# yoraish/mmd

Hardware: AMD Instinct MI355X
Metric: guided trajectories/sec (H=64, 100 denoise steps), 32-robot Empty map (higher is better)
Workload: dtype f32 (f16x2 split on the fp16 MFMA pipe: every fp32 product as 3 fp16 MFMAs, fp32 accumulate)

## Files before the change

mmd_amd/csrc/guide.hip:

```cpp
#include <hip/hip_runtime.h>

#include <atomic>
#include <cmath>

#include "../../include/mmd_amd.h"
#include "../../include/mmd_amd_debug.h"
#include "bins_dev.h"
#include "common.h"
#include "guide_dev.h"

namespace mmd {

__device__ __forceinline__ float clip_scale(float gx, float gy, float gz, float gw, float max_norm) {
  const float ax = gx + 1e-6f, ay = gy + 1e-6f, az = gz + 1e-6f, aw = gw + 1e-6f;
  const float n2 = ax * ax + ay * ay + az * az + aw * aw;
  return fminf(max_norm * __builtin_amdgcn_rsqf(n2), 1.f);
}

__device__ __forceinline__ bool clip_grad(const GuideDev& g, float& gx, float& gy, float& gz, float& gw) {
  if (g.clip_rule == 0) {
    const float sc = clip_scale(gx, gy, gz, gw, g.max_norm);
    gx = sc * gx; gy = sc * gy; gz = sc * gz; gw = sc * gw;
    return sc < 1.f;
  } else if (g.clip_rule == 1) {
    const float m = g.max_value;
    const bool on = fabsf(gx) > m || fabsf(gy) > m || fabsf(gz) > m || fabsf(gw) > m;
    gx = fminf(fmaxf(gx, -m), m); gy = fminf(fmaxf(gy, -m), m); gz = fminf(fmaxf(gz, -m), m); gw = fminf(fmaxf(gw, -m), m);
    return on;
  }
  return false;
}
__device__ __forceinline__ bool clip_grad(const GuideDev& g, float& gx, float& gy) {
  float z = 0.f, w = 0.f;
  return clip_grad(g, gx, gy, z, w);
}

__device__ __forceinline__ float lane_prev(float v) {
  return __builtin_bit_cast(float, __builtin_amdgcn_update_dpp(0, __builtin_bit_cast(int, v), 0x138, 0xf, 0xf, true));
}
__device__ __forceinline__ float lane_next(float v) {
  return __builtin_bit_cast(float, __builtin_amdgcn_update_dpp(0, __builtin_bit_cast(int, v), 0x130, 0xf, 0xf, true));
}

constexpr int LDS_SLOTS_SMALL = 40;
constexpr int LDS_SLOTS_MAX = 144;

__device__ __forceinline__ float rsq_pos(float d2) { return __builtin_amdgcn_rsqf(fmaxf(d2, 1e-30f)); }

typedef float f32x2g __attribute__((ext_vector_type(2)));
struct Acc4 { f32x2g a0, a1, a2, a3; };
__device__ __forceinline__ Acc4 acc4_zero() {
  const f32x2g z = {0.f, 0.f};
  return Acc4{z, z, z, z};
}
__device__ __forceinline__ f32x2g acc4_total(const Acc4& r) {
  return f32x2g{(r.a0.x + r.a1.x) + (r.a2.x + r.a3.x), (r.a0.y + r.a1.y) + (r.a2.y + r.a3.y)};
}
__device__ __forceinline__ f32x2g cons_term(f32x2g a, f32x2g p, f32x2g q, float r2) {
  const float dx = p.x - q.x, dy = p.y - q.y;
  const float d2 = __builtin_fmaf(dx, dx, dy * dy);
  const float m = (d2 > r2) ? 0.f : rsq_pos(d2);
  return f32x2g{__builtin_fmaf(-dx, m, a.x), __builtin_fmaf(-dy, m, a.y)};
}
template <bool COMPACT> struct ConsTab;
template <> struct ConsTab<false> {
  const float4* tab;
  float r2;
  __device__ __forceinline__ f32x2g add(f32x2g a, f32x2g p, int slot, int t) const {
    const float4 c = tab[slot * H + t];
    return cons_term(a, p, f32x2g{c.x, c.y}, c.w);
  }
};
template <> struct ConsTab<true> {
  const float2* tab;
  float r2;
  __device__ __forceinline__ f32x2g add(f32x2g a, f32x2g p, int slot, int t) const {
    const float2 c = tab[slot * H + t];
    return cons_term(a, p, f32x2g{c.x, c.y}, r2);
  }
};
template <class TAB>
__device__ __forceinline__ void cons_accumulate4(Acc4& acc, const TAB& tab, int first, int n, int rel, int t, f32x2g p) {
  auto one = [&](int k, int slot) {
    if (k == 0) acc.a0 = tab.add(acc.a0, p, slot, t);
    else if (k == 1) acc.a1 = tab.add(acc.a1, p, slot, t);
    else if (k == 2) acc.a2 = tab.add(acc.a2, p, slot, t);
    else acc.a3 = tab.add(acc.a3, p, slot, t);
  };
  int i = 0;
  for (; i < n && ((rel + i) & 3); ++i) one((rel + i) & 3, first + i);
#pragma unroll 2
  for (; i + 3 < n; i += 4) {
    acc.a0 = tab.add(acc.a0, p, first + i, t);
    acc.a1 = tab.add(acc.a1, p, first + i + 1, t);
    acc.a2 = tab.add(acc.a2, p, first + i + 2, t);
    acc.a3 = tab.add(acc.a3, p, first + i + 3, t);
  }
  for (int k = 0; i < n; ++i, ++k) one(k, first + i);
}
template <class TAB>
__device__ __forceinline__ f32x2g cons_accumulate1(f32x2g a, const TAB& tab, int first, int n, int rel, int k, int t, f32x2g p) {
#pragma unroll 4
  for (int j = (k - rel) & 3; j < n; j += 4) a = tab.add(a, p, first + j, t);
  return a;
}

struct GroupMeta {
  static constexpr bool kOneGroup = false;
  int s0[2], s1[2];
  float w[2];
  int grp0, n;
  __device__ __forceinline__ void load(const GuideDev& g, int g0, int g1) {
    grp0 = g0;
    n = min(g1 - g0, 2);
#pragma unroll
    for (int k = 0; k < 2; ++k) {
      s0[k] = s1[k] = 0;
      w[k] = 0.f;
      if (k < n) {
        s0[k] = __builtin_amdgcn_readfirstlane(g.grp_slot_off[g0 + k]);
        s1[k] = __builtin_amdgcn_readfirstlane(g.grp_slot_off[g0 + k + 1]);
        w[k] = __builtin_bit_cast(float, __builtin_amdgcn_readfirstlane(__builtin_bit_cast(int, g.grp_weight[g0 + k])));
      }
    }
  }
  __device__ __forceinline__ void bounds(const GuideDev& g, int grp, int& a, int& b) const {
    const int k = grp - grp0;
    if (k == 0 && n > 0) { a = s0[0]; b = s1[0]; }
    else if (k == 1 && n > 1) { a = s0[1]; b = s1[1]; }
    else { a = __builtin_amdgcn_readfirstlane(g.grp_slot_off[grp]); b = __builtin_amdgcn_readfirstlane(g.grp_slot_off[grp + 1]); }
  }
  __device__ __forceinline__ float weight(const GuideDev& g, int grp) const {
    const int k = grp - grp0;
    return (k == 0 && n > 0) ? w[0] : (k == 1 && n > 1) ? w[1] : g.grp_weight[grp];
  }
};

template <bool DUMP = false, class GROUPSUM, class GROUPW>
__device__ __forceinline__ float4 guide_grad(const GuideDev& g, float4 xn, int t, const float4* __restrict__ grid,
                                             int grp0, int grp1, GROUPSUM group_sum, GROUPW group_weight, unsigned int* tr = nullptr) {
  unsigned int flags = 0;
  float xu[4];
  const float xv[4] = {xn.x, xn.y, xn.z, xn.w};
#pragma unroll
  for (int d = 0; d < 4; ++d) {
    float v = fminf(fmaxf(xv[d], -1.f), 1.f);
    if constexpr (DUMP) flags |= (fabsf(xv[d]) > 1.f ? 1u : 0u) << (16 + d);
    v = (v + 1.f) / 2.f;
    xu[d] = v * g.nscale[d] + g.nmin[d];
  }
  const float px = xu[0], py = xu[1], vx = xu[2], vy = xu[3];
  const bool interior = t > 0 && t < H - 1;

  int ix = (int)floorf((px - g.lo[0]) / g.dim[0] * (float)g.nx);
  int iy = (int)floorf((py - g.lo[1]) / g.dim[1] * (float)g.ny);
  ix = min(max(ix, 0), g.nx - 1);
  iy = min(max(iy, 0), g.ny - 1);
  const float4 cell0 = g.n_grids > 0 ? grid[(size_t)ix * g.ny + iy] : make_float4(1e30f, 0.f, 0.f, 0.f);

  float wsx, wsy;
  {
    const float d0 = px - g.ws_min[0], d1 = py - g.ws_min[1], d2 = g.ws_max[0] - px, d3 = g.ws_max[1] - py;
    float best = fmaxf(g.margin - d0, 0.f), gx = -1.f, gy = 0.f;
    float v = fmaxf(g.margin - d1, 0.f);
    if (v > best) { best = v; gx = 0.f; gy = -1.f; }
    v = fmaxf(g.margin - d2, 0.f);
    if (v > best) { best = v; gx = 1.f; gy = 0.f; }
    v = fmaxf(g.margin - d3, 0.f);
    if (v > best) { best = v; gx = 0.f; gy = 1.f; }
    if (!(best > 0.f)) { gx = 0.f; gy = 0.f; }
    if constexpr (DUMP) {
      const unsigned arg = gx < 0.f ? 0u : gy < 0.f ? 1u : gx > 0.f ? 2u : 3u;
      if (best > 0.f) flags |= 1u << 4 | arg << 5;
    }
    const bool clipped = clip_grad(g, gx, gy);
    if constexpr (DUMP) flags |= (clipped ? 1u : 0u) << 9;
    wsx = g.w_coll * gx; wsy = g.w_coll * gy;
  }
  float gpx, gpy, gpz, gpw;
  {
    const float npx = lane_next(px), npy = lane_next(py), nvx = lane_next(vx), nvy = lane_next(vy);
    float wpx = 0.f, wpy = 0.f, wvx = 0.f, wvy = 0.f;
    if (t < H - 1) {
      const float epx = npx - (px + g.dt * vx), epy = npy - (py + g.dt * vy);
      const float evx = nvx - vx, evy = nvy - vy;
      wpx = 2.f * (g.m1 * epx + g.m2 * evx);
      wpy = 2.f * (g.m1 * epy + g.m2 * evy);
      wvx = 2.f * (g.m2 * epx + g.m3 * evx);
      wvy = 2.f * (g.m2 * epy + g.m3 * evy);
    }
    const float lpx = lane_prev(wpx), lpy = lane_prev(wpy), lvx = lane_prev(wvx), lvy = lane_prev(wvy);
    float gx = lpx - wpx, gy = lpy - wpy;
    float gz = lvx - (g.dt * wpx + wvx), gw = lvy - (g.dt * wpy + wvy);
    const bool clipped = clip_grad(g, gx, gy, gz, gw);
    if constexpr (DUMP) flags |= (clipped ? 1u : 0u) << 10;
    gpx = g.w_smooth * gx; gpy = g.w_smooth * gy;
    gpz = g.w_smooth * gz; gpw = g.w_smooth * gw;
  }
  float cx = 0.f, cy = 0.f;
  for (int grp = grp0; grp < grp1; ++grp) {
    const f32x2g gs = group_sum(grp, f32x2g{px, py});
    float gx = gs.x, gy = gs.y;
    const bool clipped = clip_grad(g, gx, gy);
    if constexpr (DUMP) {
      const int k = grp - grp0, s0 = g.grp_slot_off[grp], s1 = g.grp_slot_off[grp + 1];
      unsigned long long mask = 0;
      unsigned int n_act = 0;
      for (int sl = s0; sl < s1; ++sl) {
        const float4 c = g.cons[(size_t)sl * H + t];
        const float dx = px - c.x, dy = py - c.y;
        const float d2 = __builtin_fmaf(dx, dx, dy * dy);
        if (!(d2 > c.w)) {
          ++n_act;
          if (sl - s0 < 64) mask |= 1ull << (sl - s0);
        }
      }
      if (k < 4) {
        tr[2 + 2 * k] = (unsigned int)mask;
        tr[3 + 2 * k] = (unsigned int)(mask >> 32);
        flags |= (clipped ? 1u : 0u) << (11 + k);
      }
      tr[10] += n_act;
    }
    const float w = group_weight(grp);
    cx += w * gx; cy += w * gy;
  }
  float ox, oy;
  {
    float best = fmaxf(g.margin - cell0.x, 0.f), gx = 0.f, gy = 0.f;
    unsigned win = 0;
    if (best > 0.f) { gx = -cell0.y; gy = -cell0.z; }
    for (int k = 1; k < g.n_grids; ++k) {
      const float4 c = grid[((size_t)k * g.nx + ix) * g.ny + iy];
      const float v = fmaxf(g.margin - c.x, 0.f);
      if (v > best) { best = v; gx = -c.y; gy = -c.z; win = (unsigned)k; }
    }
    if (g.n_xs + g.n_xb > 0) {
      float ex, ey;
      const float v = fmaxf(g.margin - extra_sdf(g.xs, g.n_xs, g.xb, g.n_xb, px, py, ex, ey), 0.f);
      if (v > best) { best = v; gx = -ex; gy = -ey; win = 7u; }
    }
    const bool clipped = clip_grad(g, gx, gy);
    if constexpr (DUMP) {
      if (best > 0.f) flags |= 1u | (win & 7u) << 1;
      flags |= (clipped ? 1u : 0u) << 8;
    }
    ox = g.w_coll * gx; oy = g.w_coll * gy;
  }
  if constexpr (DUMP) {
    tr[0] = (unsigned int)(ix * g.ny + iy);
    tr[1] = flags | (unsigned int)min(grp1 - grp0, 15) << 20;
  }
  float tx = ((ox + wsx) + gpx) + cx, ty = ((oy + wsy) + gpy) + cy;
  float tz = gpz, tw = gpw;
  if (!interior) { tx = ty = tz = tw = 0.f; }
  return make_float4(-tx, -ty, -tz, -tw);
}


template <bool COMPACT, int NT>
__device__ __forceinline__ void stage_cons(const GuideDev& g, int robot, int lds_slots, float4* lds_cons, int& lds_slot0, int& lds_n) {
  lds_slot0 = __builtin_amdgcn_readfirstlane(g.grp_slot_off[g.robot_grp_off[robot]]);
  lds_n = min(__builtin_amdgcn_readfirstlane(g.grp_slot_off[g.robot_grp_off[robot + 1]]) - lds_slot0, lds_slots);
  const float4* src = g.cons + (size_t)lds_slot0 * H;
  if constexpr (COMPACT) {
    float2* dst = reinterpret_cast<float2*>(lds_cons);
    for (int i = threadIdx.x; i < lds_n * H; i += NT) {
      const float4 c = src[i];
      dst[i] = c.z < 0.f ? make_float2(1e30f, 1e30f) : make_float2(c.x, c.y);
    }
  } else {
    for (int i = threadIdx.x; i < lds_n * H; i += NT) lds_cons[i] = src[i];
  }
}

template <bool COMPACT, class ACC>
__device__ __forceinline__ void group_slots(const GuideDev& g, const GroupMeta& gm, int grp, const float4* lds_cons, int lds_slot0, int lds_n,
                                            ACC acc) {
  int s0, s1;
  gm.bounds(g, grp, s0, s1);
  const int l0 = min(max(s0 - lds_slot0, 0), lds_n), l1 = min(max(s1 - lds_slot0, 0), lds_n);
  if (l1 > l0) {
    if constexpr (COMPACT) acc(ConsTab<true>{reinterpret_cast<const float2*>(lds_cons), g.uniform_r2}, l0, l1 - l0, lds_slot0 + l0 - s0);
    else acc(ConsTab<false>{lds_cons, 0.f}, l0, l1 - l0, lds_slot0 + l0 - s0);
  }
  const int g0 = lds_n > 0 ? max(s0, lds_slot0 + lds_n) : s0;
  if (s1 > g0) acc(ConsTab<false>{g.cons, 0.f}, g0, s1 - g0, g0 - s0);
}

__device__ __forceinline__ float4 model_update(StepDev s, float4 v, const float4* eps, size_t idx) {
  if (s.do_model)
    v = s.ddim == 2 ? ddim_update_x0(v, eps[idx], s.a_t, s.b_t, s.c1, s.c2)
        : s.ddim ? ddim_update(v, eps[idx], s.a_t, s.b_t, s.c1, s.c2) : ddpm_posterior_mean(v, eps[idx], s.a_t, s.b_t, s.c1, s.c2);
  return v;
}

template <bool DUMP, class META = GroupMeta, class GROUPSUM>
__device__ __forceinline__ void guide_iterations(const GuideDev& g, const StepDev& s, int robot, int t, size_t idx, float4& v, bool is_hard,
                                                 float4 hv, bool store, GROUPSUM group_sum) {
  const int map = g.robot_map ? g.robot_map[robot] : 0;
  const float4* grid = g.grids + (size_t)map * g.n_grids * g.nx * g.ny;
  int grp0 = 0, grp1 = 0;
  if constexpr (META::kOneGroup) {
    grp1 = 1;
  } else if (g.robot_grp_off) {
    grp0 = __builtin_amdgcn_readfirstlane(g.robot_grp_off[robot]);
    grp1 = __builtin_amdgcn_readfirstlane(g.robot_grp_off[robot + 1]);
  }
  META gm;
  if constexpr (META::kOneGroup) gm.w = group_sum.weight;
  gm.load(g, grp0, grp1);
  for (int it = 0; it < s.n_guide_steps; ++it) {
    unsigned int* tr = nullptr;
    if constexpr (DUMP) {
      tr = s.trace + ((size_t)it * s.guide_chain_stride + idx) * MMD_TRACE_WORDS;
      for (int w = 0; w < MMD_TRACE_WORDS; ++w) tr[w] = 0u;
    }
    const float4 gr = guide_grad<DUMP>(g, v, t, grid, grp0, grp1, [&](int grp, f32x2g p) { return group_sum(gm, grp, p); },
                                       [&](int grp) { return gm.weight(g, grp); }, tr);
    v.x = __builtin_fmaf(s.grad_scale, gr.x, v.x); v.y = __builtin_fmaf(s.grad_scale, gr.y, v.y);
    v.z = __builtin_fmaf(s.grad_scale, gr.z, v.z); v.w = __builtin_fmaf(s.grad_scale, gr.w, v.w);
    if (is_hard) v = hv;
    if (s.guide_chain && store) s.guide_chain[(size_t)it * s.guide_chain_stride + idx] = v;
  }
}

__device__ __forceinline__ void step_finish(const StepDev& s, float4* x, const float4* noise, float4* chain, size_t idx, int robot,
                                            int samples_per_robot, float4& v, bool is_hard, const float4& hv) {
  if (s.do_noise) v = add_step_noise(v, noise ? noise[idx] : traj_normal4(s.seed, s.robot_seeds, s.draw, s.traj_base, idx, robot, samples_per_robot), s.sigma, s.noise_std_extra);
  if (is_hard) v = hv;
  x[idx] = v;
  if (chain) chain[idx] = v;
}

template <int WPB, bool COMPACT, bool DUMP = false>
__global__ __launch_bounds__(WPB * 64) void ddpm_guide_kernel(GuideDev g, StepDev s, int lds_slots, float4* __restrict__ x,
                                                         const float4* __restrict__ eps,
                                                         const float4* __restrict__ noise, float4* __restrict__ chain,
                                                         const float4* __restrict__ hard,
                                                         int samples_per_robot) {
  extern __shared__ __attribute__((aligned(16))) float4 lds_cons[];
  const int t = threadIdx.x & 63;
  const int traj_b = s.traj0 + blockIdx.x * WPB;
  const int traj = traj_b + (threadIdx.x >> 6);
  const bool valid = traj < s.traj_end;

  int lds_slot0 = 0, lds_n = 0;
  if (s.do_guide && g.robot_grp_off) {
    const int rb0 = traj_b / samples_per_robot;
    const int rb1 = min(traj_b + WPB - 1, s.traj_end - 1) / samples_per_robot;
    if (rb0 == rb1) stage_cons<COMPACT, WPB * 64>(g, rb0, lds_slots, lds_cons, lds_slot0, lds_n);
  }
  __syncthreads();
  if (!valid) return;

  const int robot = traj / samples_per_robot;
  const size_t idx = (size_t)traj * H + t;
  float4 v = model_update(s, x[idx], eps, idx);
  float4 hv = v;
  const bool is_hard = hard_row(s.hard_rows, s.n_hard, hard, robot, t, hv);
  if constexpr (DUMP) {
    if (s.mu_out) s.mu_out[idx] = v;
  }
  if (s.do_guide)
    guide_iterations<DUMP>(g, s, robot, t, idx, v, is_hard, hv, true, [&](const GroupMeta& gm, int grp, f32x2g p) {
      Acc4 acc = acc4_zero();
      group_slots<COMPACT>(g, gm, grp, lds_cons, lds_slot0, lds_n,
                           [&](const auto& tab, int first, int n, int rel) { cons_accumulate4(acc, tab, first, n, rel, t, p); });
      return acc4_total(acc);
    });
  step_finish(s, x, noise, chain, idx, robot, samples_per_robot, v, is_hard, hv);
}

constexpr int COOP_XCH_BYTES = 2 * 4 * H * 8;
template <bool COMPACT>
__global__ __launch_bounds__(256) void ddpm_guide_coop_kernel(GuideDev g, StepDev s, int lds_slots, float4* __restrict__ x,
                                                              const float4* __restrict__ eps, const float4* __restrict__ noise,
                                                              float4* __restrict__ chain, const float4* __restrict__ hard,
                                                              int samples_per_robot) {
  extern __shared__ __attribute__((aligned(16))) float4 lds_cons[];
  const int t = threadIdx.x & 63, wave = __builtin_amdgcn_readfirstlane(threadIdx.x >> 6);
  const int traj = s.traj0 + blockIdx.x;
  const int robot = traj / samples_per_robot;
  float2* const xch = reinterpret_cast<float2*>(reinterpret_cast<char*>(lds_cons) + (size_t)lds_slots * H * (COMPACT ? 8 : 16));
  int lds_slot0 = 0, lds_n = 0;
  if (s.do_guide && g.robot_grp_off) stage_cons<COMPACT, 256>(g, robot, lds_slots, lds_cons, lds_slot0, lds_n);
  __syncthreads();
  const size_t idx = (size_t)traj * H + t;
  float4 v = model_update(s, x[idx], eps, idx);
  float4 hv = v;
  const bool is_hard = hard_row(s.hard_rows, s.n_hard, hard, robot, t, hv);
  if (s.do_guide) {
    int parity = 0;
    guide_iterations<false>(g, s, robot, t, idx, v, is_hard, hv, wave == 0, [&](const GroupMeta& gm, int grp, f32x2g p) {
      f32x2g a = {0.f, 0.f};
      group_slots<COMPACT>(g, gm, grp, lds_cons, lds_slot0, lds_n,
                           [&](const auto& tab, int first, int n, int rel) { a = cons_accumulate1(a, tab, first, n, rel, wave, t, p); });
      float2* const slot = xch + parity * 4 * H;
      slot[wave * H + t] = make_float2(a.x, a.y);
      __syncthreads();
      parity ^= 1;
      const float2 q0 = slot[t], q1 = slot[H + t], q2 = slot[2 * H + t], q3 = slot[3 * H + t];
      return acc4_total(Acc4{f32x2g{q0.x, q0.y}, f32x2g{q1.x, q1.y}, f32x2g{q2.x, q2.y}, f32x2g{q3.x, q3.y}});
    });
  }
  if (wave != 0) return;
  step_finish(s, x, noise, chain, idx, robot, samples_per_robot, v, is_hard, hv);
}


struct OneGroup {
  static constexpr bool kOneGroup = true;
  float w;
  __device__ __forceinline__ void load(const GuideDev&, int, int) {}
  __device__ __forceinline__ float weight(const GuideDev&, int) const { return w; }
};

struct BinnedSum {
  const mmd_cons_bins& b;
  int t, self;
  float r2, weight;
  __device__ __forceinline__ f32x2g operator()(const OneGroup&, int, f32x2g p) const {
    const CellList cl = own_cell_list(b, t, p.x, p.y);
    const float4 none = make_float4(0.f, 0.f, __builtin_bit_cast(float, self), 0.f);
    Acc4 acc = acc4_zero();
    const int last = max(cl.e1 - 1, 0);
    for (int e = cl.e0; __builtin_amdgcn_ballot_w64(e < cl.e1) != 0; e += 4) {
      float4 c[4];
#pragma unroll
      for (int j = 0; j < 4; ++j) {
        const float4 l = cl.ent[min(e + j, last)];
        c[j] = e + j < cl.e1 ? l : none;
      }
#pragma unroll
      for (int j = 0; j < 4; ++j) {
        const int id = __builtin_bit_cast(int, c[j].z);
        const int k = (id - (id > self ? 1 : 0)) & 3;
        f32x2g a = k == 0 ? acc.a0 : k == 1 ? acc.a1 : k == 2 ? acc.a2 : acc.a3;
        a = cons_term(a, p, f32x2g{c[j].x, c[j].y}, id != self ? r2 : -1.f);
        acc.a0 = k == 0 ? a : acc.a0;
        acc.a1 = k == 1 ? a : acc.a1;
        acc.a2 = k == 2 ? a : acc.a2;
        acc.a3 = k == 3 ? a : acc.a3;
      }
    }
    return acc4_total(acc);
  }
};

__global__ __launch_bounds__(256) void ddpm_guide_binned_kernel(GuideDev g, StepDev s, mmd_cons_bins b, float4* __restrict__ x,
                                                                const float4* __restrict__ eps, const float4* __restrict__ noise,
                                                                float4* __restrict__ chain, const float4* __restrict__ hard,
                                                                int samples_per_robot) {
  const int t = threadIdx.x & 63;
  const int traj = s.traj0 + blockIdx.x * 4 + (threadIdx.x >> 6);
  if (traj >= s.traj_end) return;
  const int robot = traj / samples_per_robot;
  const size_t idx = (size_t)traj * H + t;
  float4 v = model_update(s, x[idx], eps, idx);
  float4 hv = v;
  const bool is_hard = hard_row(s.hard_rows, s.n_hard, hard, robot, t, hv);
  if (s.do_guide)
    guide_iterations<false, OneGroup>(g, s, robot, t, idx, v, is_hard, hv, true,
                                      BinnedSum{b, t, b.robot0 + robot, b.radius * fabsf(b.radius), b.weight});
  step_finish(s, x, noise, chain, idx, robot, samples_per_robot, v, is_hard, hv);
}

__global__ void init_kernel(float4* __restrict__ x, float4* __restrict__ chain, const float4* __restrict__ hard,
                            unsigned long long hard_rows, int draw_noise, unsigned long long seed,
                            const unsigned long long* __restrict__ robot_seeds, long long traj_base, int n_traj, int samples_per_robot) {
  const size_t idx = (size_t)blockIdx.x * blockDim.x + threadIdx.x;
  if (idx >= (size_t)n_traj * H) return;
  const int t = idx % H;
  const int robot = (idx / H) / samples_per_robot;
  float4 v = draw_noise ? traj_normal4(seed, robot_seeds, 0xFFFFFFFFu, traj_base, idx, robot, samples_per_robot) : x[idx];
  float4 hv;
  if (hard_row(hard_rows, __popcll(hard_rows), hard, robot, t, hv)) v = hv;
  x[idx] = v;
  if (chain) chain[idx] = v;
}

__global__ void q_sample_kernel(float4* __restrict__ x, const float4* __restrict__ x0, const float4* __restrict__ noise,
                                float a, float b, unsigned long long seed, unsigned int draw, long long traj_base,
                                size_t n_pts) {
  const size_t idx = (size_t)blockIdx.x * blockDim.x + threadIdx.x;
  if (idx >= n_pts) return;
  const float4 z = noise ? noise[idx] : normal4(seed, draw, (unsigned long long)traj_base * H + idx);
  const float4 s = x0[idx];
  x[idx] = make_float4(a * s.x + b * z.x, a * s.y + b * z.y, a * s.z + b * z.z, a * s.w + b * z.w);
}

__global__ void cross_condition_kernel(float4* __restrict__ x1, float4* __restrict__ x2, float4* __restrict__ c1,
                                       float4* __restrict__ c2, int ind1, int ind2, float4 rel, float4 bnd,
                                       const float4* __restrict__ by_robot, int spr, int n_traj) {
  const int b = blockIdx.x * blockDim.x + threadIdx.x;
  if (b >= n_traj) return;
  if (by_robot) {
    rel = by_robot[(size_t)(b / spr) * 2];
    bnd = by_robot[(size_t)(b / spr) * 2 + 1];
  }
  const float4 v2 = x2[(size_t)b * H + ind2];
  float4 v1;
  v1.x = fminf(v2.x + rel.x, bnd.x); v1.y = fminf(v2.y + rel.y, bnd.y);
  v1.z = fminf(v2.z + rel.z, bnd.z); v1.w = fminf(v2.w + rel.w, bnd.w);
  x1[(size_t)b * H + ind1] = v1;
  float4 w;
  w.x = fmaxf(v1.x - rel.x, -bnd.x); w.y = fmaxf(v1.y - rel.y, -bnd.y);
  w.z = fmaxf(v1.z - rel.z, -bnd.z); w.w = fmaxf(v1.w - rel.w, -bnd.w);
  x2[(size_t)b * H + ind2] = w;
  if (c1) c1[(size_t)b * H + ind1] = v1;
  if (c2) c2[(size_t)b * H + ind2] = w;
}

int fill_guide(const mmd_guide_desc* d, GuideDev& g) {
  MMD_REQUIRE(d->n_grids == 0 || (d->sdf_grids_dev && d->grid_nx >= 1 && d->grid_ny >= 1), "guide: SDF grid missing");
  if (d->cons_bins) {
    MMD_REQUIRE(!d->cons_ell_dev, "guide: cons_bins together with an ELL table (cons_ell_dev) is not supported");
    if (int rc = check_cons_bins(d->cons_bins)) return rc;
  }
  for (int k = 0; k < 4; ++k) { g.nmin[k] = d->norm_min[k]; g.nscale[k] = d->norm_max[k] - d->norm_min[k]; }
  for (int k = 0; k < 2; ++k) {
    g.lo[k] = d->limits_lo[k];
    g.dim[k] = fabsf(d->limits_hi[k] - d->limits_lo[k]);
    g.ws_min[k] = d->ws_min[k]; g.ws_max[k] = d->ws_max[k];
  }
  g.nx = d->grid_nx; g.ny = d->grid_ny; g.n_grids = d->n_grids;
  g.grids = reinterpret_cast<const float4*>(d->sdf_grids_dev);
  g.robot_map = d->robot_map_dev;
  g.margin = d->margin; g.dt = d->dt; g.w_coll = d->weight_collision; g.w_smooth = d->weight_smoothness;
  g.max_norm = d->max_grad_norm;
  MMD_REQUIRE(d->clip_grad_rule >= 0 && d->clip_grad_rule <= 2, "guide: clip_grad_rule must be 0 (norm), 1 (value) or 2 (off)");
  g.clip_rule = d->clip_grad_rule;
  g.max_value = d->max_grad_value;
  const double dt = d->dt, qc = 1.0 / ((double)d->sigma_gp * d->sigma_gp);
  g.m1 = (float)(12.0 / (dt * dt * dt) * qc);
  g.m2 = (float)(-6.0 / (dt * dt) * qc);
  g.m3 = (float)(4.0 / dt * qc);
  g.max_slots = d->max_slots_per_robot > 0 ? d->max_slots_per_robot : LDS_SLOTS_SMALL;
  g.uniform_r2 = d->cons_uniform_radius > 0.f ? d->cons_uniform_radius * fabsf(d->cons_uniform_radius) : 0.f;
  g.xs = reinterpret_cast<const float4*>(d->extra_spheres_dev); g.n_xs = d->extra_spheres_dev ? d->n_extra_spheres : 0;
  g.xb = reinterpret_cast<const float4*>(d->extra_boxes_dev); g.n_xb = d->extra_boxes_dev ? d->n_extra_boxes : 0;
  g.cons = reinterpret_cast<const float4*>(d->cons_ell_dev);
  g.grp_slot_off = d->grp_slot_off_dev; g.grp_weight = d->grp_weight_dev; g.robot_grp_off = d->robot_grp_off_dev;
  if (!g.cons || !g.grp_slot_off || !g.grp_weight) g.robot_grp_off = nullptr;
  return 0;
}

constexpr int kCoopMaxTrajDefault = 512;

int launch_step(const GuideDev& g, StepDev s, float* x, const float* eps, const float* noise, float* chain,
                const float* hard, int traj0, int n_traj, int spr, hipStream_t st, const mmd_cons_bins* bins) {
  s.traj0 = traj0;
  s.traj_end = traj0 + n_traj;
  if (bins && s.do_guide) {
    hipLaunchKernelGGL(ddpm_guide_binned_kernel, dim3((n_traj + 3) / 4), dim3(256), 0, st, g, s, *bins, (float4*)x, (const float4*)eps,
                       (const float4*)noise, (float4*)chain, (const float4*)hard, spr);
    return 0;
  }
  const bool guided = s.do_guide && g.robot_grp_off;
  const bool compact = guided && g.uniform_r2 > 0.f;
  const int bytes_per_slot = H * (compact ? 8 : 16);
  const int small = LDS_SLOTS_SMALL * (compact ? 2 : 1), big = LDS_SLOTS_MAX * (compact ? 2 : 1);
  auto launch = [&](auto kern, int grid, int block, size_t lds_bytes, int slots) {
    hipLaunchKernelGGL(kern, dim3(grid), dim3(block), lds_bytes, st, g, s, slots, (float4*)x, (const float4*)eps, (const float4*)noise,
                       (float4*)chain, (const float4*)hard, spr);
  };
  if (s.trace) {
    launch(ddpm_guide_kernel<4, false, true>, (n_traj + 3) / 4, 256, 0, 0);
  } else if (guided && n_traj <= (s.coop_max > 0 ? s.coop_max : s.coop_max < 0 ? 0 : kCoopMaxTrajDefault)) {
    const int fit = 60 * 1024 / bytes_per_slot;
    const int slots = g.max_slots < fit ? g.max_slots : fit;
    launch(compact ? ddpm_guide_coop_kernel<true> : ddpm_guide_coop_kernel<false>, n_traj, 256,
           (size_t)slots * bytes_per_slot + COOP_XCH_BYTES, slots);
  } else if (guided && g.max_slots > small && spr % 8 == 0 && traj0 % 8 == 0) {
    const int slots = g.max_slots < big ? g.max_slots : big;
    static std::atomic<unsigned long long> attr_devices{0};
    int dev = 0;
    (void)hipGetDevice(&dev);
    const unsigned long long bit = 1ull << (dev & 63);
    if (!(attr_devices.load(std::memory_order_acquire) & bit)) {
      (void)hipFuncSetAttribute(reinterpret_cast<const void*>(&ddpm_guide_kernel<8, false>),
                                hipFuncAttributeMaxDynamicSharedMemorySize, LDS_SLOTS_MAX * H * 16);
      (void)hipFuncSetAttribute(reinterpret_cast<const void*>(&ddpm_guide_kernel<8, true>),
                                hipFuncAttributeMaxDynamicSharedMemorySize, LDS_SLOTS_MAX * H * 16);
      attr_devices.fetch_or(bit, std::memory_order_release);
    }
    launch(compact ? ddpm_guide_kernel<8, true> : ddpm_guide_kernel<8, false>, (n_traj + 7) / 8, 512, (size_t)slots * bytes_per_slot, slots);
  } else {
    const int slots = guided ? small : 0;
    launch(compact ? ddpm_guide_kernel<4, true> : ddpm_guide_kernel<4, false>, (n_traj + 3) / 4, 256, (size_t)slots * bytes_per_slot, slots);
  }
  return 0;
}

void launch_cross(float* x1, float* x2, float* c1, float* c2, int ind1, int ind2, const float* rel, const float* bnd,
                  const float* by_robot, int spr, int n_traj, hipStream_t st) {
  hipLaunchKernelGGL(cross_condition_kernel, dim3((n_traj + 255) / 256), dim3(256), 0, st, (float4*)x1, (float4*)x2,
                     (float4*)c1, (float4*)c2, ind1, ind2, make_float4(rel[0], rel[1], rel[2], rel[3]),
                     make_float4(bnd[0], bnd[1], bnd[2], bnd[3]), (const float4*)by_robot, spr > 0 ? spr : 1, n_traj);
}

int launch_init(float* x, float* chain, const float* hard, unsigned long long hard_rows, int draw, unsigned long long seed,
                const unsigned long long* robot_seeds, long long traj_base, int n_traj, int spr, hipStream_t st) {
  const size_t n = (size_t)n_traj * H;
  hipLaunchKernelGGL(init_kernel, dim3((unsigned)((n + 255) / 256)), dim3(256), 0, st, (float4*)x, (float4*)chain,
                     (const float4*)hard, hard_rows, draw, seed, robot_seeds, traj_base, n_traj, spr);
  return 0;
}

}

using namespace mmd;

extern "C" {

int mmd_guide_steps(const mmd_guide_desc* d, float* x_dev, const float* hard_dev, uint64_t hard_rows, int n_robots,
                    int samples_per_robot, int n_steps, float* chain_dev, void* stream) {
  MMD_REQUIRE(d && x_dev && hard_dev, "mmd_guide_steps: NULL argument");
  GuideDev g{};
  if (int rc = fill_guide(d, g)) return rc;
  StepDev s{};
  s.do_guide = 1; s.n_guide_steps = n_steps; s.hard_rows = hard_rows; s.n_hard = __builtin_popcountll(hard_rows); s.grad_scale = 1.f;
  s.guide_chain = reinterpret_cast<float4*>(chain_dev);
  s.guide_chain_stride = (long long)n_robots * samples_per_robot * H;
  launch_step(g, s, x_dev, nullptr, nullptr, nullptr, hard_dev, 0, n_robots * samples_per_robot, samples_per_robot,
              (hipStream_t)stream, d->cons_bins);
  MMD_HIP_CHECK(hipGetLastError());
  return 0;
}

int mmd_q_sample(float* x_dev, const float* x_start_dev, const float* noise_dev, float a, float b, uint64_t seed,
                 uint32_t draw_index, int64_t traj_index_base, int n_traj, void* stream) {
  MMD_REQUIRE(x_dev && x_start_dev && n_traj >= 1, "mmd_q_sample: bad arguments");
  const size_t n = (size_t)n_traj * H;
  hipLaunchKernelGGL(q_sample_kernel, dim3((unsigned)((n + 255) / 256)), dim3(256), 0, (hipStream_t)stream,
                     (float4*)x_dev, (const float4*)x_start_dev, (const float4*)noise_dev, a, b,
                     (unsigned long long)seed, draw_index, (long long)traj_index_base, n);
  MMD_HIP_CHECK(hipGetLastError());
  return 0;
}

int mmd_cross_condition(float* x1_dev, float* x2_dev, int ind1, int ind2, const float* rel, const float* boundary,
                        int n_traj, void* stream) {
  MMD_REQUIRE(x1_dev && x2_dev && rel && boundary, "mmd_cross_condition: NULL argument");
  MMD_REQUIRE(ind1 >= 0 && ind1 < H && ind2 >= 0 && ind2 < H, "row index out of range");
  launch_cross(x1_dev, x2_dev, nullptr, nullptr, ind1, ind2, rel, boundary, nullptr, 1, n_traj, (hipStream_t)stream);
  MMD_HIP_CHECK(hipGetLastError());
  return 0;
}

}
```

Before: 97190.

## Pad first staged constraint group to multiple of eight for branch-free trip loop

When staging a robot's constraints into LDS, the first group is padded with inert sentinel slots up to a multiple of eight, and later groups are shifted past the padding. The common first group then runs a fixed 8-wide loop with no alignment prologue or remainder tail. The LDS slot count for the 8-wave kernel is rounded up to make room for the padding. This costs extra LDS and some wasted sentinel evaluations, and adds offset bookkeeping to the other groups.

Result: no change. 97670 (median of 3 runs) (+0.5%).

```diff
diff --git a/mmd_amd/csrc/guide.hip b/mmd_amd/csrc/guide.hip
--- a/mmd_amd/csrc/guide.hip
+++ b/mmd_amd/csrc/guide.hip
@@ -103,6 +103,18 @@
 #pragma unroll 4
   for (int j = (k - rel) & 3; j < n; j += 4) a = tab.add(a, p, first + j, t);
   return a;
+}
+template <class TAB>
+__device__ __forceinline__ void cons_accumulate_trips(Acc4& acc, const TAB& tab, int n_trips, int t, f32x2g p) {
+  for (int i = 0; i < 8 * n_trips; i += 8) {
+#pragma unroll
+    for (int j = 0; j < 8; j += 4) {
+      acc.a0 = tab.add(acc.a0, p, i + j, t);
+      acc.a1 = tab.add(acc.a1, p, i + j + 1, t);
+      acc.a2 = tab.add(acc.a2, p, i + j + 2, t);
+      acc.a3 = tab.add(acc.a3, p, i + j + 3, t);
+    }
+  }
 }
 
 struct GroupMeta {
@@ -258,33 +270,54 @@
 }
 
 
-template <bool COMPACT, int NT>
-__device__ __forceinline__ void stage_cons(const GuideDev& g, int robot, int lds_slots, float4* lds_cons, int& lds_slot0, int& lds_n) {
-  lds_slot0 = __builtin_amdgcn_readfirstlane(g.grp_slot_off[g.robot_grp_off[robot]]);
-  lds_n = min(__builtin_amdgcn_readfirstlane(g.grp_slot_off[g.robot_grp_off[robot + 1]]) - lds_slot0, lds_slots);
-  const float4* src = g.cons + (size_t)lds_slot0 * H;
+struct Staged { int slot0 = 0, n = 0, trips = 0, pad = 0; };
+
+template <bool COMPACT, int NT, bool PAD>
+__device__ __forceinline__ Staged stage_cons(const GuideDev& g, int robot, int lds_slots, float4* lds_cons) {
+  Staged st;
+  const int grp = __builtin_amdgcn_readfirstlane(g.robot_grp_off[robot]);
+  st.slot0 = __builtin_amdgcn_readfirstlane(g.grp_slot_off[grp]);
+  st.n = min(__builtin_amdgcn_readfirstlane(g.grp_slot_off[g.robot_grp_off[robot + 1]]) - st.slot0, lds_slots);
+  int n0 = st.n;
+  if constexpr (PAD) {
+    if (st.n > 0) {
+      n0 = min(__builtin_amdgcn_readfirstlane(g.grp_slot_off[grp + 1]) - st.slot0, st.n);
+      const int pad = -n0 & 7;
+      if (n0 > 0 && st.n + pad <= lds_slots) { st.pad = pad; st.trips = (n0 + pad) >> 3; }
+    }
+  }
+  const float4* src = g.cons + (size_t)st.slot0 * H;
+  const int split = n0 * H, shift = st.pad * H;
   if constexpr (COMPACT) {
     float2* dst = reinterpret_cast<float2*>(lds_cons);
-    for (int i = threadIdx.x; i < lds_n * H; i += NT) {
+    for (int i = threadIdx.x; i < st.n * H; i += NT) {
       const float4 c = src[i];
-      dst[i] = c.z < 0.f ? make_float2(1e30f, 1e30f) : make_float2(c.x, c.y);
-    }
+      dst[i < split ? i : i + shift] = c.z < 0.f ? make_float2(1e30f, 1e30f) : make_float2(c.x, c.y);
+    }
+    for (int i = threadIdx.x; i < shift; i += NT) dst[split + i] = make_float2(1e30f, 1e30f);
   } else {
-    for (int i = threadIdx.x; i < lds_n * H; i += NT) lds_cons[i] = src[i];
-  }
-}
-
-template <bool COMPACT, class ACC>
-__device__ __forceinline__ void group_slots(const GuideDev& g, const GroupMeta& gm, int grp, const float4* lds_cons, int lds_slot0, int lds_n,
-                                            ACC acc) {
+    for (int i = threadIdx.x; i < st.n * H; i += NT) lds_cons[i < split ? i : i + shift] = src[i];
+    for (int i = threadIdx.x; i < shift; i += NT) lds_cons[split + i] = make_float4(0.f, 0.f, -1.f, -1.f);
+  }
+  return st;
+}
+
+template <bool COMPACT, class ACC, class TRIPS>
+__device__ __forceinline__ void group_slots(const GuideDev& g, const GroupMeta& gm, int grp, const float4* lds_cons, const Staged& st, ACC acc,
+                                            TRIPS trips) {
   int s0, s1;
   gm.bounds(g, grp, s0, s1);
-  const int l0 = min(max(s0 - lds_slot0, 0), lds_n), l1 = min(max(s1 - lds_slot0, 0), lds_n);
-  if (l1 > l0) {
-    if constexpr (COMPACT) acc(ConsTab<true>{reinterpret_cast<const float2*>(lds_cons), g.uniform_r2}, l0, l1 - l0, lds_slot0 + l0 - s0);
-    else acc(ConsTab<false>{lds_cons, 0.f}, l0, l1 - l0, lds_slot0 + l0 - s0);
-  }
-  const int g0 = lds_n > 0 ? max(s0, lds_slot0 + lds_n) : s0;
+  if (st.trips > 0 && s0 == st.slot0) {
+    if constexpr (COMPACT) trips(ConsTab<true>{reinterpret_cast<const float2*>(lds_cons), g.uniform_r2}, st.trips);
+    else trips(ConsTab<false>{lds_cons, 0.f}, st.trips);
+  } else {
+    const int l0 = min(max(s0 - st.slot0, 0), st.n), l1 = min(max(s1 - st.slot0, 0), st.n);
+    if (l1 > l0) {
+      if constexpr (COMPACT) acc(ConsTab<true>{reinterpret_cast<const float2*>(lds_cons), g.uniform_r2}, l0 + st.pad, l1 - l0, st.slot0 + l0 - s0);
+      else acc(ConsTab<false>{lds_cons, 0.f}, l0 + st.pad, l1 - l0, st.slot0 + l0 - s0);
+    }
+  }
+  const int g0 = st.n > 0 ? max(s0, st.slot0 + st.n) : s0;
   if (s1 > g0) acc(ConsTab<false>{g.cons, 0.f}, g0, s1 - g0, g0 - s0);
 }
 
@@ -345,11 +378,11 @@
   const int traj = traj_b + (threadIdx.x >> 6);
   const bool valid = traj < s.traj_end;
 
-  int lds_slot0 = 0, lds_n = 0;
+  Staged st;
   if (s.do_guide && g.robot_grp_off) {
     const int rb0 = traj_b / samples_per_robot;
     const int rb1 = min(traj_b + WPB - 1, s.traj_end - 1) / samples_per_robot;
-    if (rb0 == rb1) stage_cons<COMPACT, WPB * 64>(g, rb0, lds_slots, lds_cons, lds_slot0, lds_n);
+    if (rb0 == rb1) st = stage_cons<COMPACT, WPB * 64, true>(g, rb0, lds_slots, lds_cons);
   }
   __syncthreads();
   if (!valid) return;
@@ -365,8 +398,9 @@
   if (s.do_guide)
     guide_iterations<DUMP>(g, s, robot, t, idx, v, is_hard, hv, true, [&](const GroupMeta& gm, int grp, f32x2g p) {
       Acc4 acc = acc4_zero();
-      group_slots<COMPACT>(g, gm, grp, lds_cons, lds_slot0, lds_n,
-                           [&](const auto& tab, int first, int n, int rel) { cons_accumulate4(acc, tab, first, n, rel, t, p); });
+      group_slots<COMPACT>(g, gm, grp, lds_cons, st,
+                           [&](const auto& tab, int first, int n, int rel) { cons_accumulate4(acc, tab, first, n, rel, t, p); },
+                           [&](const auto& tab, int n_trips) { cons_accumulate_trips(acc, tab, n_trips, t, p); });
       return acc4_total(acc);
     });
   step_finish(s, x, noise, chain, idx, robot, samples_per_robot, v, is_hard, hv);
@@ -383,8 +417,8 @@
   const int traj = s.traj0 + blockIdx.x;
   const int robot = traj / samples_per_robot;
   float2* const xch = reinterpret_cast<float2*>(reinterpret_cast<char*>(lds_cons) + (size_t)lds_slots * H * (COMPACT ? 8 : 16));
-  int lds_slot0 = 0, lds_n = 0;
-  if (s.do_guide && g.robot_grp_off) stage_cons<COMPACT, 256>(g, robot, lds_slots, lds_cons, lds_slot0, lds_n);
+  Staged st;
+  if (s.do_guide && g.robot_grp_off) st = stage_cons<COMPACT, 256, false>(g, robot, lds_slots, lds_cons);
   __syncthreads();
   const size_t idx = (size_t)traj * H + t;
   float4 v = model_update(s, x[idx], eps, idx);
@@ -394,8 +428,9 @@
     int parity = 0;
     guide_iterations<false>(g, s, robot, t, idx, v, is_hard, hv, wave == 0, [&](const GroupMeta& gm, int grp, f32x2g p) {
       f32x2g a = {0.f, 0.f};
-      group_slots<COMPACT>(g, gm, grp, lds_cons, lds_slot0, lds_n,
-                           [&](const auto& tab, int first, int n, int rel) { a = cons_accumulate1(a, tab, first, n, rel, wave, t, p); });
+      group_slots<COMPACT>(g, gm, grp, lds_cons, st,
+                           [&](const auto& tab, int first, int n, int rel) { a = cons_accumulate1(a, tab, first, n, rel, wave, t, p); },
+                           [](const auto&, int) {});
       float2* const slot = xch + parity * 4 * H;
       slot[wave * H + t] = make_float2(a.x, a.y);
       __syncthreads();
@@ -573,7 +608,7 @@
     launch(compact ? ddpm_guide_coop_kernel<true> : ddpm_guide_coop_kernel<false>, n_traj, 256,
            (size_t)slots * bytes_per_slot + COOP_XCH_BYTES, slots);
   } else if (guided && g.max_slots > small && spr % 8 == 0 && traj0 % 8 == 0) {
-    const int slots = g.max_slots < big ? g.max_slots : big;
+    const int slots = ((g.max_slots + 7) & ~7) < big ? (g.max_slots + 7) & ~7 : big;
     static std::atomic<unsigned long long> attr_devices{0};
     int dev = 0;
     (void)hipGetDevice(&dev);
```
